# kalakris/stomp_motion_planner_icra2011

Measured on AMD Instinct MI355X. Metric: STOMP iterations/sec (7-DOF, 100 wp, K=512, 256³ SDF) at 1/2/4/8 GPUs, higher is better.
Workload: dtype f64; 1 GPU; cfg2: 7-DOF, 100 wp (N=99), K=512 (512/GPU), K_r=0, 256^3 SDF, S=49 spheres; global_rollouts=512, rollouts_per_gpu=512, parallelism=rollout shard x1

## Files before the change

stomp_motion_planner_icra2011_amd/csrc/device_fk.h:

```cpp
#pragma once

#include "kernels.h"
#include "stomp_math.h"

namespace stomp {

struct Frame {
    double R[9];
    double p[3];
};

__device__ __forceinline__ void rotmul(const double* A, const double* B, double* C)
{
#pragma unroll
    for (int i = 0; i < 3; ++i)
#pragma unroll
        for (int j = 0; j < 3; ++j)
            C[3 * i + j] = A[3 * i + 0] * B[0 + j] + A[3 * i + 1] * B[3 + j] + A[3 * i + 2] * B[6 + j];
}

__device__ __forceinline__ void pose_rotation(const DevSegment& sg, double st, double ct, double* R)
{
    const double* a = sg.axis;
    const double vt = 1.0 - ct;
    const double m_vt_0 = vt * a[0], m_vt_1 = vt * a[1], m_vt_2 = vt * a[2];
    const double m_st_0 = a[0] * st, m_st_1 = a[1] * st, m_st_2 = a[2] * st;
    const double m_vt_0_1 = m_vt_0 * a[1], m_vt_0_2 = m_vt_0 * a[2], m_vt_1_2 = m_vt_1 * a[2];
    double Rq[9];
    Rq[0] = ct + m_vt_0 * a[0];
    Rq[1] = -m_st_2 + m_vt_0_1;
    Rq[2] = m_st_1 + m_vt_0_2;
    Rq[3] = m_st_2 + m_vt_0_1;
    Rq[4] = ct + m_vt_1 * a[1];
    Rq[5] = -m_st_0 + m_vt_1_2;
    Rq[6] = -m_st_1 + m_vt_0_2;
    Rq[7] = m_st_0 + m_vt_1_2;
    Rq[8] = ct + m_vt_2 * a[2];
    if (sg.rot_identity) {
#pragma unroll
        for (int k = 0; k < 9; ++k) R[k] = Rq[k];
    } else {
#pragma unroll
        for (int i = 0; i < 3; ++i)
#pragma unroll
            for (int j = 0; j < 3; ++j)
                R[3 * i + j] = sg.rot[3 * i + 0] * Rq[0 + j] + sg.rot[3 * i + 1] * Rq[3 + j] + sg.rot[3 * i + 2] * Rq[6 + j];
    }
}

__device__ __forceinline__ void compose(const DevSegment& sg, const Frame* parent, double st, double ct, Frame& out)
{
    Frame pose;
    if (sg.q_index >= 0) {
        const double* a = sg.axis;
        const double vt = 1.0 - ct;
        const double m_vt_0 = vt * a[0], m_vt_1 = vt * a[1], m_vt_2 = vt * a[2];
        const double m_st_0 = a[0] * st, m_st_1 = a[1] * st, m_st_2 = a[2] * st;
        const double m_vt_0_1 = m_vt_0 * a[1], m_vt_0_2 = m_vt_0 * a[2], m_vt_1_2 = m_vt_1 * a[2];
        double Rq[9];
        Rq[0] = ct + m_vt_0 * a[0];
        Rq[1] = -m_st_2 + m_vt_0_1;
        Rq[2] = m_st_1 + m_vt_0_2;
        Rq[3] = m_st_2 + m_vt_0_1;
        Rq[4] = ct + m_vt_1 * a[1];
        Rq[5] = -m_st_0 + m_vt_1_2;
        Rq[6] = -m_st_1 + m_vt_0_2;
        Rq[7] = m_st_0 + m_vt_1_2;
        Rq[8] = ct + m_vt_2 * a[2];
        if (sg.rot_identity) {
#pragma unroll
            for (int k = 0; k < 9; ++k) pose.R[k] = Rq[k];
        } else {
            rotmul(sg.rot, Rq, pose.R);
        }
    } else {
#pragma unroll
        for (int k = 0; k < 9; ++k) pose.R[k] = sg.rot[k];
    }
#pragma unroll
    for (int k = 0; k < 3; ++k) pose.p[k] = sg.trans[k];
    if (!parent) {
        out = pose;
        return;
    }
    if (sg.q_index < 0 && sg.rot_identity) {
#pragma unroll
        for (int k = 0; k < 9; ++k) out.R[k] = parent->R[k];
    } else {
        rotmul(parent->R, pose.R, out.R);
    }
#pragma unroll
    for (int i = 0; i < 3; ++i)
        out.p[i] = parent->R[3 * i + 0] * pose.p[0] + parent->R[3 * i + 1] * pose.p[1] +
                   parent->R[3 * i + 2] * pose.p[2] + parent->p[i];
}

__device__ __forceinline__ void apply(const double* R, const double* P, const double* v, double* o)
{
#pragma unroll
    for (int i = 0; i < 3; ++i) o[i] = R[3 * i + 0] * v[0] + R[3 * i + 1] * v[1] + R[3 * i + 2] * v[2] + P[i];
}

__device__ __forceinline__ void fk_op(const DevSegment& sg, int base, int save, double st, double ct, Frame& C,
                                      Frame& S0, Frame& S1)
{
    Frame nf;
    if (base == kBaseChain) {
        compose(sg, &C, st, ct, nf);
    } else if (base == kBaseRoot) {
        compose(sg, nullptr, st, ct, nf);
    } else {
        Frame P;
#pragma unroll
        for (int k = 0; k < 9; ++k) P.R[k] = base == 0 ? S0.R[k] : S1.R[k];
#pragma unroll
        for (int k = 0; k < 3; ++k) P.p[k] = base == 0 ? S0.p[k] : S1.p[k];
        compose(sg, &P, st, ct, nf);
    }
    C = nf;
    if (save >= 0) {
#pragma unroll
        for (int k = 0; k < 9; ++k) {
            S0.R[k] = save == 0 ? C.R[k] : S0.R[k];
            S1.R[k] = save == 1 ? C.R[k] : S1.R[k];
        }
#pragma unroll
        for (int k = 0; k < 3; ++k) {
            S0.p[k] = save == 0 ? C.p[k] : S0.p[k];
            S1.p[k] = save == 1 ? C.p[k] : S1.p[k];
        }
    }
}

// ... 50 lines not shown
```

stomp_motion_planner_icra2011_amd/csrc/engine_create.cpp:

```cpp
#include "engine_internal.h"

#include <algorithm>
#include <cstdlib>

using namespace stomp;

namespace {

bool sphere_thresholds(double radius, double clearance, double res, int* zero_lim, int* col_lim)
{
    if (!(radius >= 0.0 && clearance > 0.0 && std::isfinite(radius) && std::isfinite(clearance))) return false;
    int zl = 65536, cl = 65536;
    bool zseen = false, cseen = false;
    for (int d2 = 0; d2 <= 65535; ++d2) {
        const double dist = std::sqrt((double)d2) * res;
        const double dd = dist - radius;
        const bool zero = dd >= clearance;
        const bool col = dist <= radius;
        if (zero && !zseen) { zl = d2; zseen = true; }
        if (!zero && zseen) return false;
        if (!col && !cseen) { cl = d2; cseen = true; }
        if (col && cseen) return false;
    }
    *zero_lim = zl;
    *col_lim = cl;
    return true;
}

int plan_fk(stomp_engine* e, const stomp_engine_desc* d, std::vector<FkOp>& ops)
{
    const int ns = d->num_segments;
    std::vector<char> needed(ns, 0);
    int prev = -1;
    for (int j = 0; j < d->num_spheres; ++j) {
        int s = d->spheres[j].segment;
        if (s < prev)
            return fail(e, STOMP_E_UNSUPPORTED,
                        "sphere list must be ordered by segment (sphere %d on segment %d after segment %d)", j, s, prev);
        prev = s;
        for (int a = s; a >= 0 && !needed[a]; a = d->segments[a].parent) needed[a] = 1;
    }
    std::vector<int> remaining(ns, 0), slot_of(ns, -1);
    for (int s = 0; s < ns; ++s)
        if (needed[s] && d->segments[s].parent >= 0) remaining[d->segments[s].parent]++;
    bool used[kSaves] = {false, false};
    const int runmax = run_max(d->num_time_steps);
    int sph = 0, cur = -1;
    for (int s = 0; s < ns; ++s) {
        if (!needed[s]) continue;
        const int p = d->segments[s].parent;
        int base;
        if (p < 0) base = kBaseRoot;
        else if (p == cur) base = kBaseChain;
        else if (slot_of[p] >= 0) base = slot_of[p];
        else return fail(e, STOMP_E_UNSUPPORTED, "FK planner: parent frame of segment %d not available", s);
        if (p >= 0 && --remaining[p] == 0 && slot_of[p] >= 0) {
            used[slot_of[p]] = false;
            slot_of[p] = -1;
        }
        int save = -1;
        if (remaining[s] >= 2) {
            for (int k = 0; k < kSaves; ++k)
                if (!used[k]) { used[k] = true; save = k; break; }
            if (save < 0) return fail(e, STOMP_E_UNSUPPORTED, "kinematic tree needs more than %d saved frames", kSaves);
            slot_of[s] = save;
        }
        cur = s;
        int b = sph;
        while (sph < d->num_spheres && d->spheres[sph].segment == s) ++sph;
        const int slot = sph > b ? e->nslots++ : -1;
        for (int j = b; j < sph; ++j) e->sphere_slot[j] = slot;
        bool first = true;
        for (int a = b; a < sph || first; a += runmax) {
            FkOp o;
            o.seg = first ? s : -1;
            o.base = first ? base : kBaseChain;
            o.save = first ? save : -1;
            o.slot = first ? slot : -1;
            o.sph_begin = std::min(a, sph);
            o.sph_end = std::min(a + runmax, sph);
            ops.push_back(o);
            first = false;
        }
    }
    return 0;
}

const char* torque_chain(const stomp_engine_desc* d, std::vector<int>& path)
{
    path.clear();
    if (!d->inertias) return "torque term needs segment inertias";
    if (d->torque_root < 0 || d->torque_root >= d->num_segments || d->torque_tip < 0 ||
        d->torque_tip >= d->num_segments)
        return "torque chain root/tip out of range";
    for (int sgi = d->torque_tip; sgi != d->torque_root; sgi = d->segments[sgi].parent) {
        if (sgi < 0 || (int)path.size() == kMaxChain) return "torque tip is not below the torque root (or chain too long)";
        path.push_back(sgi);
    }
    std::reverse(path.begin(), path.end());
    int nj = 0;
    for (int sgi : path)
        if (d->segments[sgi].q_index >= 0 && d->segments[sgi].q_index != nj++) return "torque chain joints must be the group joints in order";
    if (nj != d->num_joints) return "torque chain joints must be the group joints in order";
    return nullptr;
}

void oc_nominal_inverse(const double* q, double* O)
{
    double x = q[0], y = q[1], z = q[2], w = q[3];
    const double l2 = x * x + y * y + z * z + w * w;
    if (std::fabs(l2 - 1.0) > 0.1f) {
        const double inv = 1.0 / std::sqrt(l2);
        x *= inv; y *= inv; z *= inv; w *= inv;
    }
    const double d = x * x + y * y + z * z + w * w;
    const double s = 2.0 / d;
    const double xs = x * s, ys = y * s, zs = z * s;
    const double wx = w * xs, wy = w * ys, wz = w * zs;
    const double xx = x * xs, xy = x * ys, xz = x * zs;
    const double yy = y * ys, yz = y * zs, zz = z * zs;
    const double M[9] = {1.0 - (yy + zz), xy - wz, xz + wy, xy + wz, 1.0 - (xx + zz), yz - wx,
                         xz - wy, yz + wx, 1.0 - (xx + yy)};
    auto cof = [&](int r1, int c1, int r2, int c2) { return M[3 * r1 + c1] * M[3 * r2 + c2] - M[3 * r1 + c2] * M[3 * r2 + c1]; };
    const double co0 = cof(1, 1, 2, 2), co1 = cof(1, 2, 2, 0), co2 = cof(1, 0, 2, 1);
    const double det = M[0] * co0 + M[1] * co1 + M[2] * co2;
    const double sc = 1.0 / det;
    O[0] = co0 * sc; O[1] = cof(0, 2, 2, 1) * sc; O[2] = cof(0, 1, 1, 2) * sc;
    O[3] = co1 * sc; O[4] = cof(0, 0, 2, 2) * sc; O[5] = cof(0, 2, 1, 0) * sc;
    O[6] = co2 * sc; O[7] = cof(0, 1, 2, 0) * sc; O[8] = cof(0, 0, 1, 1) * sc;
}

struct HostTables {
    std::vector<double> LT, MT, QT;
    std::vector<DevSegment> segs;
    std::vector<DevSphere> sph;
    std::vector<int> slot_sph, has_lim;
    std::vector<double> jmin, jmax;
};

struct AbandonEngine {
    void operator()(stomp_engine* e) const
    {
        g_last_error = e->err;
        release(e);
        delete e;
    }
};

int world_of(const stomp_engine_desc* d) { return d->world_size > 0 ? d->world_size : 1; }

int validate_desc(const stomp_engine_desc* d)
{
    if (d->abi_version != STOMP_ENGINE_ABI_VERSION)
        return fail(nullptr, STOMP_E_INVALID, "abi_version %d != %d", d->abi_version, STOMP_ENGINE_ABI_VERSION);
    if (d->num_joints <= 0 || d->num_joints > kMaxJoints)
        return fail(nullptr, STOMP_E_INVALID, "num_joints must be in [1, %d]", kMaxJoints);
    if (d->num_time_steps <= 0 || d->num_time_steps > 256)
        return fail(nullptr, STOMP_E_INVALID, "num_time_steps must be in [1, 256]");
    if (d->num_rollouts <= 0) return fail(nullptr, STOMP_E_INVALID, "num_rollouts must be positive");
    if (d->num_reused_rollouts < 0 || d->num_reused_rollouts >= d->num_rollouts)
        return fail(nullptr, STOMP_E_INVALID, "Number of reused rollouts must be strictly less than number of rollouts.");
    if (d->num_orientation_constraints < 0 || (d->num_orientation_constraints > 0 && !d->orientation_constraints))
        return fail(nullptr, STOMP_E_INVALID, "invalid orientation constraints");
    for (int c = 0; c < d->num_orientation_constraints; ++c)
        if (d->orientation_constraints[c].segment < 0 || d->orientation_constraints[c].segment >= d->num_segments)
            return fail(nullptr, STOMP_E_INVALID, "orientation constraint %d: bad segment", c);
    if (d->num_segments <= 0 || !d->segments || (d->num_spheres > 0 && !d->spheres) || !d->joints || !d->noise_stddev ||
        !d->noise_decay || !d->start || !d->goal || !d->grid.data)
// ... 10 lines not shown
            return fail(nullptr, STOMP_E_INVALID, "sphere %d: bad segment", j);
        int zl, cl;
        if (!sphere_thresholds(d->spheres[j].radius, d->spheres[j].clearance, d->grid.resolution, &zl, &cl))
            return fail(nullptr, STOMP_E_INVALID, "sphere %d: radius / clearance not finite and positive", j);
    }
    if (d->torque_cost_weight > 1e-9) {
        std::vector<int> path;
        if (const char* why = torque_chain(d, path)) return fail(nullptr, STOMP_E_UNSUPPORTED, "%s", why);
    }
    const int world = world_of(d);
    if (world > 1) {
        if (!d->comm_id) return fail(nullptr, STOMP_E_INVALID, "world_size > 1 needs a comm_id");
        if (d->rank < 0 || d->rank >= world)
            return fail(nullptr, STOMP_E_INVALID, "rank %d outside [0, world_size %d)", d->rank, world);
        if (d->num_rollouts % (world * kSumBlock) != 0)
            return fail(nullptr, STOMP_E_INVALID, "num_rollouts must be a multiple of 64 * world_size");
        if (!kWithRccl && !is_local_comm_id(d->comm_id))
            return fail(nullptr, STOMP_E_UNSUPPORTED, "built without RCCL (use stomp_comm_local_id)");
    }
    return 0;
}

int open_engine(stomp_engine* e, const stomp_engine_desc* d)
{
    e->device = d->device;
    if (hipSetDevice(d->device) != hipSuccess) return fail(e, STOMP_E_DEVICE, "hipSetDevice(%d) failed", d->device);
    if (d->stream) {
        e->stream = (hipStream_t)d->stream;
    } else {
        hipStreamCreateWithFlags(&e->stream, hipStreamNonBlocking);
        e->own_stream = true;
    }
    const int world = world_of(d);
    e->J = d->num_joints; e->N = d->num_time_steps; e->Nall = e->N + 2 * kPad;
    e->K = d->num_rollouts; e->Kr = d->num_reused_rollouts;
    e->world = world; e->rank = world > 1 ? d->rank : 0;
    e->K_loc = e->K / world; e->first = e->rank * e->K_loc;
    e->S = d->num_spheres; e->nseg = d->num_segments; e->seed = d->seed;
    e->disc = d->discretization; e->w_smooth = d->smoothness_cost_weight; e->w_obs = d->obstacle_cost_weight;
    e->w_con = d->constraint_cost_weight; e->w_tq = d->torque_cost_weight;
    for (int r = 0; r < 3; ++r) e->smooth[r] = d->smoothness_costs[r];
    e->use_cum = d->use_cumulative_costs; e->max_it = d->max_iterations;
    e->max_it_cf = d->max_iterations_after_collision_free;
    e->sig_std.assign(d->noise_stddev, d->noise_stddev + e->J);
    e->sig_dec.assign(d->noise_decay, d->noise_decay + e->J);
    e->start.assign(d->start, d->start + e->J);
    e->goal.assign(d->goal, d->goal + e->J);
    return 0;
}

int choose_decomposition(stomp_engine* e, const stomp_engine_desc* d, bool local_id)
{
    const int world = e->world;
    if (e->K_loc > kSumBlock * 64) return fail(e, STOMP_E_INVALID, "at most %d rollouts per device", kSumBlock * 64);
    e->pre_on = (e->Kr == 0 || world == 1) && e->J <= 16;
    const bool can = e->pre_on && e->Kr == 0 && e->K <= kSumBlock * 64;
    const char* sm = std::getenv("STOMP_SHARD_MODE");
    if (world > 1 && sm && std::strcmp(sm, "gather") == 0 && !can)
        return fail(e, STOMP_E_UNSUPPORTED, "STOMP_SHARD_MODE=gather needs the pregen rows in the rollout launch "
                                            "and no reused rollouts (K_r = %d, J = %d)", e->Kr, e->J);
    const char* sim = std::getenv("STOMP_DEBUG_GATHER_RANKS");
    const int W = (world == 1 && sim) ? std::atoi(sim) : 0;
    if (W > 1 && can && e->K % (W * kSumBlock) == 0) {
        e->gather = true;
        e->K_loc = e->K / W;
    } else if (world > 1 && can) {
        e->gather = sm ? std::strcmp(sm, "gather") == 0 : (size_t)e->K * e->N * sizeof(double) <= (1u << 20);
    }
    const char* cl = std::getenv("STOMP_DEBUG_CALIBRATE_LOCAL");
    e->calibrate = world > 1 && can && !sm && (!local_id || (cl && cl[0] == '1'));
    if (e->calibrate) e->gather = true;
    e->rows = e->gather ? e->K : e->K_loc;
    e->row0 = (e->gather && world > 1) ? e->first : 0;
    const char* dbg = std::getenv("STOMP_DEBUG_SHARDED_MODES");
    e->split_modes = (world > 1 && !e->gather) ||
                     (world == 1 && !e->gather && dbg && dbg[0] == '1' && d->num_rollouts % kSumBlock == 0 &&
                      d->num_reused_rollouts == 0);
    return 0;
}

int setup_tables(stomp_engine* e, const stomp_engine_desc* d, HostTables& t)
{
    e->sphere_slot.assign(std::max(e->S, 1), 0);
    if (int rc = plan_fk(e, d, e->ops)) return rc;
    SetupInput si;
    si.J = e->J; si.N = e->N; si.discretization = e->disc;
    for (int r = 0; r < 3; ++r) si.smoothness_costs[r] = e->smooth[r];
    si.ridge_factor = d->ridge_factor;
    for (int j = 0; j < e->J; ++j) si.joint_cost.push_back(d->joints[j].joint_cost);
    si.start = e->start; si.goal = e->goal;
    std::string msg = compute_setup(si, e->su);
    if (!msg.empty()) return fail(e, STOMP_E_INVALID, "%s", msg.c_str());

    const int J = e->J, N = e->N;
    t.LT.assign((size_t)(N + kMatPadRows) * N, 0.0);
    t.MT.assign((size_t)(N + kMatPadRows) * N, 0.0);
    t.QT.resize((size_t)J * N * N);
    for (int i = 0; i < N; ++i)
        for (int k = 0; k < N; ++k) {
            t.LT[(size_t)k * N + i] = e->su.L[(size_t)i * N + k];
            t.MT[(size_t)k * N + i] = e->su.M[(size_t)i * N + k];
        }
    for (int j = 0; j < J; ++j)
        for (int i = 0; i < N; ++i)
            for (int k = 0; k < N; ++k)
                t.QT[((size_t)j * N + k) * N + i] = e->su.Qinv[((size_t)j * N + i) * N + k];
    t.segs.resize(e->nseg);
    for (int s = 0; s < e->nseg; ++s) {
        const stomp_segment& g = d->segments[s];
        DevSegment& o = t.segs[s];
        o.parent = g.parent; o.q_index = g.q_index;
        std::memcpy(o.rot, g.rot, sizeof g.rot);
        o.rot_identity = g.rot[0] == 1.0 && g.rot[1] == 0.0 && g.rot[2] == 0.0 && g.rot[3] == 0.0 &&
                         g.rot[4] == 1.0 && g.rot[5] == 0.0 && g.rot[6] == 0.0 && g.rot[7] == 0.0 &&
                         g.rot[8] == 1.0;
        o.pad_ = 0;
        std::memcpy(o.trans, g.trans, sizeof g.trans);
        std::memcpy(o.axis, g.axis, sizeof g.axis);
    }
    t.sph.resize(std::max(e->S, 1));
    for (int j = 0; j < e->S; ++j) {
        const stomp_sphere& g = d->spheres[j];
        DevSphere& o = t.sph[j];
        o.slot = e->sphere_slot[j];
        o.radius = g.radius; o.clearance = g.clearance;
        o.inv_clearance = 1.0 / g.clearance;
        std::memcpy(o.pos, g.pos, sizeof g.pos);
        sphere_thresholds(g.radius, g.clearance, d->grid.resolution, &o.zero_lim, &o.col_lim);
        o.pad_ = 0;
    }
    t.has_lim.resize(J);
    t.jmin.resize(J);
    t.jmax.resize(J);
    for (int j = 0; j < J; ++j) {
        t.has_lim[j] = d->joints[j].has_limits;
        t.jmin[j] = d->joints[j].min;
        t.jmax[j] = d->joints[j].max;
    }
    t.slot_sph.assign(e->nslots + 1, e->S);
    for (int j = e->S - 1; j >= 0; --j) t.slot_sph[e->sphere_slot[j]] = j;
    return 0;
}

int alloc_reuse_buffers(stomp_engine* e)
{
    const int J = e->J, N = e->N;
    if (e->world == 1 && e->Kr > 0) {
        if (int rc = dev_alloc(e, &e->d_reuse_costs, (size_t)e->K + 1)) return rc;
        if (int rc = dev_alloc(e, &e->d_reuse_count, 1)) return rc;
        const char* no_spec = std::getenv("STOMP_DEBUG_NO_SPEC");
        if (!(no_spec && std::strcmp(no_spec, "1") == 0)) {
            const size_t n = ((size_t)e->K + 1) * J * N;
            if (int rc = dev_alloc(e, &e->d_spec_params, n)) return rc;
            if (int rc = dev_alloc(e, &e->d_spec_noise, n)) return rc;
            if (int rc = dev_alloc(e, &e->d_spec_ctl, n)) return rc;
            e->spec_on = true;
        }
        const char* no_fuse = std::getenv("STOMP_DEBUG_NO_PICK_FUSE");
        e->pick_fuse = !(no_fuse && std::strcmp(no_fuse, "1") == 0);
    }
    if (e->world > 1 && e->Kr > 0) {
        const size_t slot = (size_t)e->Kr * ((size_t)J * N + N);
        if (int rc = dev_alloc(e, &e->d_tot_loc, (size_t)e->K_loc)) return rc;
        if (int rc = dev_alloc(e, &e->d_tot_all, (size_t)e->K)) return rc;
        if (int rc = dev_alloc(e, &e->d_tot_x, 1)) return rc;
        if (int rc = dev_alloc(e, &e->d_sel, (size_t)e->Kr)) return rc;
        if (int rc = dev_alloc(e, &e->d_slot, slot)) return rc;
        if (int rc = dev_alloc(e, &e->d_slot_all, slot * e->world)) return rc;
    }
    return 0;
}

int alloc_buffers(stomp_engine* e, const stomp_engine_desc* d, const HostTables& tab)
{
    const int J = e->J, N = e->N;
    if (int rc = upload(e, &e->d_QT, tab.QT.data(), tab.QT.size())) return rc;
    if (int rc = upload(e, &e->d_LT, tab.LT.data(), tab.LT.size())) return rc;
    if (int rc = upload(e, &e->d_MT, tab.MT.data(), tab.MT.size())) return rc;
    if (int rc = upload(e, &e->d_theta, e->su.theta.data(), e->su.theta.size())) return rc;
    if (int rc = upload(e, &e->d_start, e->start.data(), e->start.size())) return rc;
    if (int rc = upload(e, &e->d_goal, e->goal.data(), e->goal.size())) return rc;
    const size_t ncell = (size_t)d->grid.nx * d->grid.ny * d->grid.nz;
    e->grid_n[0] = d->grid.nx; e->grid_n[1] = d->grid.ny; e->grid_n[2] = d->grid.nz;
    if (d->grid.data_on_device) {
        e->d_sdf = (uint16_t*)d->grid.data;
        e->d_sdf_caller = d->grid.data;
    } else {
        if (int rc = upload(e, &e->d_sdf, d->grid.data, ncell)) return rc;
    }
    const size_t KJN = (size_t)e->rows * J * N;
    if (int rc = dev_alloc(e, &e->d_params, KJN)) return rc;
    if (int rc = dev_alloc(e, &e->d_noise, KJN)) return rc;
    if (int rc = dev_alloc(e, &e->d_control, KJN)) return rc;
    if (int rc = dev_alloc(e, &e->d_prob, KJN)) return rc;
    if (int rc = dev_alloc(e, &e->d_state, (size_t)e->rows * N)) return rc;
    if (e->gather && hipMemsetAsync(e->d_state, 0, sizeof(double) * e->rows * N, e->stream) != hipSuccess)
        return fail(e, STOMP_E_DEVICE, "memset failed");
    if (e->Kr > 0) {
        if (int rc = dev_alloc(e, &e->d_params_b, KJN)) return rc;
        if (int rc = dev_alloc(e, &e->d_noise_b, KJN)) return rc;
        if (int rc = dev_alloc(e, &e->d_control_b, KJN)) return rc;
        if (int rc = dev_alloc(e, &e->d_state_b, (size_t)e->K_loc * N)) return rc;
// ... 65 lines not shown
    t.torque = d->torque_cost_weight > 1e-9 ? 1 : 0;
    t.nchain = (int)cs.size();
    t.chain = d_chain;
    for (int k = 0; k < 3; ++k) t.g[k] = d->gravity[k];
    if (t.torque) e->terms_on = true;
    e->torque_stats = true;
    return 0;
}

int build_constraints(stomp_engine* e, const stomp_engine_desc* d)
{
    if (d->num_orientation_constraints <= 0) return 0;
    std::vector<OcDev> oc(d->num_orientation_constraints);
    for (int c = 0; c < d->num_orientation_constraints; ++c) {
        const stomp_orientation_constraint& in = d->orientation_constraints[c];
        OcDev& o = oc[c];
        std::vector<int> path;
        for (int sgi = in.segment; sgi >= 0; sgi = d->segments[sgi].parent) path.push_back(sgi);
        if ((int)path.size() > kMaxChain)
            return fail(e, STOMP_E_UNSUPPORTED, "constraint segment deeper than %d", kMaxChain);
        std::reverse(path.begin(), path.end());
        o.seg = in.segment; o.body_fixed = in.body_fixed ? 1 : 0; o.path_len = (int)path.size();
        for (size_t k = 0; k < path.size(); ++k) o.path[k] = path[k];
        oc_nominal_inverse(in.orientation, o.ninv);
        o.tol[0] = in.absolute_roll_tolerance; o.tol[1] = in.absolute_pitch_tolerance;
        o.tol[2] = in.absolute_yaw_tolerance; o.weight = in.weight;
        o.rw = o.pw = o.yw = 1.0;
        if (o.tol[1] >= M_PI) o.pw = 0.0;
        if (o.tol[0] >= M_PI) o.rw = 0.0;
        if (o.tol[2] >= M_PI) o.yw = 0.0;
    }
    OcDev* d_oc;
    if (int rc = upload(e, &d_oc, oc.data(), oc.size())) return rc;
    e->terms.noc = (int)oc.size();
    e->terms.oc = d_oc;
    e->terms_on = true;
    return 0;
}

int build_terms(stomp_engine* e, const stomp_engine_desc* d, const HostTables& tab)
{
    const int J = e->J, N = e->N;
    if (int rc = build_torque_chain(e, d, tab)) return rc;
    if (int rc = build_constraints(e, d)) return rc;
    if (e->terms_on || e->torque_stats) {
        TermsModel& t = e->terms;
        t.J = J; t.N = N;
        const double invTime = 1.0 / e->disc, invTime2 = 1.0 / (e->disc * e->disc);
        for (int k = 0; k < 7; ++k) {
            t.cv[k] = invTime * kDiffRules[0][k];
            t.ca[k] = invTime2 * kDiffRules[1][k];
        }
        t.start = e->d_start; t.goal = e->d_goal;
        t.w_con = e->w_con; t.w_tq = e->w_tq;
        if (terms_lds_bytes(t) > 160 * 1024) {
            if (e->terms_on)
                return fail(e, STOMP_E_UNSUPPORTED, "state-terms kernel needs %zu B of LDS", terms_lds_bytes(t));
            e->torque_stats = false;
        }
        if (getenv("STOMP_DEBUG_LEAN_PRINT"))
            fprintf(stderr, "stomp: terms J %d N %d nchain %d noc %d torque %d stats %d, k_terms<%d>, LDS %zu B, "
                            "opt-in %d\n", J, N, t.nchain, t.noc, t.torque, e->torque_stats ? 1 : 0, N <= 128 ? 128 : 256,
                    terms_lds_bytes(t), terms_lds_bytes(t) > 64 * 1024 ? 1 : 0);
        if (e->terms_on)
            if (int rc = dev_alloc(e, &e->d_terms_traj, (size_t)e->K_loc * J * N)) return rc;
        if (e->torque_stats) {
            e->tq_model = t;
            e->tq_model.torque = 1;
            e->tq_model.noc = 0;
            if (int rc = dev_alloc(e, &e->d_tq, (size_t)N)) return rc;
            if (int rc = dev_alloc(e, &e->d_tq_state, (size_t)N)) return rc;
        }
    }
    if (int rc = dev_alloc(e, &e->d_delta, (size_t)J * N)) return rc;
    e->pi_weight = e->w_smooth;
    if (hipDeviceGetAttribute(&e->wall_khz, hipDeviceAttributeWallClockRate, d->device) != hipSuccess) e->wall_khz = 0;
    return 0;
}

int choose_layout(stomp_engine* e, const stomp_engine_desc* d, const HostTables& tab)
{
    const int J = e->J, N = e->N;
    DevModel& m = e->model;
    m.J = J; m.N = N; m.Nall = e->Nall; m.S = e->S; m.nops = (int)e->ops.size(); m.nseg = e->nseg;
    m.nslots = e->nslots;
    m.sph_chunk = 1;
    for (const FkOp& o : e->ops) m.sph_chunk = std::max(m.sph_chunk, o.sph_end - o.sph_begin);
    if (m.sph_chunk * N > 65535)
        return fail(e, STOMP_E_UNSUPPORTED, "%d spheres on one segment x %d waypoints exceed 16-bit pair ids",
                    m.sph_chunk, N);
    m.nsaves = 0;
    for (const FkOp& o : e->ops) m.nsaves = std::max(m.nsaves, o.save + 1);
    int last_joint = -1, first_save = (int)e->ops.size();
    for (int i = 0; i < (int)e->ops.size(); ++i) {
        const FkOp& o = e->ops[i];
        if (o.seg >= 0 && tab.segs[o.seg].q_index >= 0) last_joint = i;
        if (o.save >= 0 && first_save == (int)e->ops.size()) first_save = i;
    }
    m.sincos_pre = m.nsaves >= 1 && J <= 12 * m.nsaves && first_save > last_joint ? 1 : 0;
    const size_t stat = rollout_static_lds();
    const size_t with_pad = rollout_lds_bytes(m, 1) + stat, without = rollout_lds_bytes(m, 0) + stat;
    int cus = 0;
    if (hipDeviceGetAttribute(&cus, hipDeviceAttributeMultiprocessorCount, d->device) != hipSuccess || cus <= 0)
        cus = 256;
    m.cus = cus;
    const int blocks = e->K_loc + 1 + (e->pre_on ? e->rows : 0) + (e->Kr > 0 && e->world == 1 ? e->K : 0);
    const int need = (blocks + cus - 1) / cus;
    m.pad_lds = (with_pad <= kRolloutLdsMax &&
                 rollout_blocks_per_cu(with_pad) >= std::min(need, rollout_blocks_per_cu(without))) ? 1 : 0;
    const size_t lds = rollout_lds_bytes(m, m.pad_lds) + stat;
    m.phased_lds = (int)rollout_phased_lds_bytes(m);
    if (getenv("STOMP_DEBUG_PHASED")) fprintf(stderr, "stomp: phased rollout LDS %d B\n", m.phased_lds);
    if (lds > kRolloutLdsMax)
        return fail(e, STOMP_E_UNSUPPORTED, "rollout kernel needs %zu B of LDS (J=%d, N=%d, S=%d, %d spheres "
                                            "on one segment), more than %zu", lds, J, N, e->S, m.sph_chunk,
                    kRolloutLdsMax);
    m.lean = 0;
    const int per_cu_full = rollout_blocks_per_cu(lds);
    int per_cu[3] = {per_cu_full, 0, 0};
    for (int lv = 1; lv <= 2; ++lv)
        if (rollout_lean_allowed(m, lv)) per_cu[lv] = rollout_blocks_per_cu(rollout_lds_bytes(m, 0, lv) + stat, lv);
    if (need > per_cu_full) {
        int best = per_cu_full;
        for (int lv = 1; lv <= 2; ++lv)
            if (per_cu[lv] > best) {
                best = per_cu[lv];
                m.lean = lv;
            }
    }
    if (const char* v = getenv("STOMP_DEBUG_LEAN")) {
        const int lv = atoi(v);
        if (lv >= 0 && lv <= 2 && rollout_lean_allowed(m, lv)) m.lean = lv;
    }
    if (getenv("STOMP_DEBUG_LEAN_PRINT"))
        fprintf(stderr, "stomp: rollout LDS full %zu / lean1 %zu / lean2 %zu B, workgroups per CU %d / %d / %d, "
                        "needed %d, layout lean %d\n", lds, rollout_lds_bytes(m, 0, 1) + stat,
                rollout_lds_bytes(m, 0, 2) + stat, per_cu[0], per_cu[1], per_cu[2], need, m.lean);
    if (!cost_supported(m)) return fail(e, STOMP_E_UNSUPPORTED, "FK program too large (%d ops, %d segments)",
                                        m.nops, m.nseg);
    return 0;
}

int upload_lds_image(stomp_engine* e, const HostTables& tab)
{
    const int J = e->J, N = e->N;
    DevModel& m = e->model;
    const RolloutLds L = rollout_lds(J, N, e->S, m.sph_chunk, m.nsaves, m.nseg, m.nops, m.nslots, 1);
    std::vector<unsigned char> img(L.total - L.sph, 0);
    auto put = [&](size_t off, const void* src, size_t bytes) {
        if (bytes) std::memcpy(img.data() + (off - L.sph), src, bytes);
    };
    std::vector<double> jlim(2 * (size_t)J);
    for (int j = 0; j < J; ++j) { jlim[2 * j] = tab.jmin[j]; jlim[2 * j + 1] = tab.jmax[j]; }
    put(L.sph, tab.sph.data(), sizeof(DevSphere) * e->S);
    put(L.seg, tab.segs.data(), sizeof(DevSegment) * tab.segs.size());
    put(L.ops, e->ops.data(), sizeof(FkOp) * e->ops.size());
    put(L.slot, tab.slot_sph.data(), sizeof(int) * tab.slot_sph.size());
    put(L.hl, tab.has_lim.data(), sizeof(int) * J);
    put(L.jlim, jlim.data(), sizeof(double) * jlim.size());
    unsigned long long* d_img;
    if (int rc = upload(e, &d_img, (const unsigned long long*)img.data(), img.size() / 8)) return rc;
    if (hipStreamSynchronize(e->stream) != hipSuccess)
        return fail(e, STOMP_E_DEVICE, "table upload failed");
    const unsigned char* base = (const unsigned char*)d_img;
    m.img = d_img;
    m.img_words = (int)(((m.pad_lds ? L.total : L.pad) - L.sph) / 8);
    m.sph = (const DevSphere*)(base + (L.sph - L.sph));
    m.segs = (const DevSegment*)(base + (L.seg - L.sph));
    m.ops = (const FkOp*)(base + (L.ops - L.sph));
    m.slot_sph = (const int*)(base + (L.slot - L.sph));
    e->d_pad_pos = (double*)(base + (L.pad - L.sph));
    m.pad_pos = e->d_pad_pos; m.sdf = e->d_sdf;
    return 0;
}

int place_field(stomp_engine* e, const stomp_engine_desc* d)
{
    DevModel& m = e->model;
    const size_t ncell = (size_t)d->grid.nx * d->grid.ny * d->grid.nz;
    const char* lay = std::getenv("STOMP_SDF_LAYOUT");
    const bool brick = lay ? std::strcmp(lay, "brick") == 0 : ncell * sizeof(uint16_t) > ((size_t)64 << 20);
    m.brick = 0;
    m.nby = (d->grid.ny + 3) / 4;
    m.nbz = (d->grid.nz + 3) / 4;
    if (!brick) return 0;
    uint16_t* bricks = nullptr;
    if (int rc = dev_alloc(e, &bricks, sdf_brick_cells(d->grid.nx, d->grid.ny, d->grid.nz))) return rc;
    launch_sdf_bricks(e->d_sdf, bricks, d->grid.nx, d->grid.ny, d->grid.nz, e->stream);
    if (hipStreamSynchronize(e->stream) != hipSuccess)
        return fail(e, STOMP_E_DEVICE, "distance-field brick layout failed");
    if (!d->grid.data_on_device) {
        auto it = std::find(e->allocs.begin(), e->allocs.end(), (void*)e->d_sdf);
        if (it != e->allocs.end()) {
            hipFree(*it);
            e->allocs.erase(it);
        }
    }
    e->d_sdf = bricks;
    m.sdf = bricks;
    m.brick = 1;
    return 0;
}

int finish_model(stomp_engine* e, const stomp_engine_desc* d)
{
    const int J = e->J, N = e->N;
    DevModel& m = e->model;
    e->terms.segs = m.segs;
    e->tq_model.segs = m.segs;
    m.nx = d->grid.nx; m.ny = d->grid.ny; m.nz = d->grid.nz;
    m.ny_d = (double)m.ny; m.nz_d = (double)m.nz;
    m.hi_x = m.nx - 1.5; m.hi_y = m.ny - 1.5; m.hi_z = m.nz - 1.5;
    m.ox = d->grid.origin[0]; m.oy = d->grid.origin[1]; m.oz = d->grid.origin[2]; m.res = d->grid.resolution;
    m.inv_res = 1.0 / d->grid.resolution;
    m.start = e->d_start; m.goal = e->d_goal;
    const double invTime = 1.0 / e->disc;
    for (int k = 0; k < 7; ++k) {
        m.vel_coef[k] = invTime * kDiffRules[0][k];
        if ((k < kVelTap0 || k > kVelTap1) && kDiffRules[0][k] != 0.0)
            return fail(e, STOMP_E_UNSUPPORTED, "velocity rule tap %d outside the kernel's stencil", k);
    }
    m.w_obs = e->w_obs; m.w_con = e->w_con; m.w_tq = e->w_tq;
    m.QT = e->d_QT;
    m.split_cap = std::max(e->K_loc + 2, m.cus / 2 + 1);
    if (int rc = dev_alloc(e, &m.split_cnt, (size_t)m.split_cap)) return rc;
    if (m.lean && m.nsaves > 0) {
        m.sv_rows = e->K_loc + 1;
        if (int rc = dev_alloc(e, &m.sv_glob, (size_t)m.sv_rows * m.nsaves * 12 * N)) return rc;
    }
    {
        const char* env = std::getenv("STOMP_DEBUG_SPLIT_MAX");
        m.split_max = env ? std::atoi(env) : 0;
        const char* xi = std::getenv("STOMP_DEBUG_XCTL_INLINE");
        m.x_ctl_inline = xi && std::strcmp(xi, "1") == 0 ? 1 : 0;
    }
    if (getenv("STOMP_DEBUG_LEAN_PRINT")) {
        const int nro = e->K_loc + 1, extra = e->pre_on ? e->rows : 0;
        const int P = rollout_split_pieces(m, nro, extra, false);
        const char* body = P ? "split" : nro <= m.cus ? (m.phased_lds > 0 ? "phased" : "wide")
                                                      : (m.lean ? "lean slot loop" : "slot loop");
        fprintf(stderr, "stomp: model J %d N %d S %d nseg %d nops %d nsaves %d sincos_pre %d sph_chunk %d lean %d "
                        "pregen %d fused_noise %d brick %d, launch of %d rollouts: %s, %d pieces, weights %s\n",
                J, N, e->S, m.nseg, m.nops, m.nsaves, m.sincos_pre, m.sph_chunk, m.lean, e->pre_on ? 1 : 0,
                J <= 16 ? 1 : 0, m.brick, nro, body, P, weights_kernel_name(e->K_loc, !e->split_modes, false));
    }
    return 0;
}

int pad_fk(stomp_engine* e)
{
    const int J = e->J, N = e->N;
    DevModel& m = e->model;
    m.pad_collision = 0;
    launch_pad_fk(m, e->d_start, e->d_goal, e->d_pad_pos, e->d_pad_cf, e->stream);
    int pad_cf = 0;
    if (hipMemcpyAsync(&pad_cf, e->d_pad_cf, sizeof(int), hipMemcpyDeviceToHost, e->stream) != hipSuccess ||
        hipStreamSynchronize(e->stream) != hipSuccess)
        return fail(e, STOMP_E_DEVICE, "padding FK failed: %s", hipGetErrorString(hipGetLastError()));
    m.pad_collision = pad_cf;
    e->pad_collision = pad_cf;
    if (hipMemcpyAsync(e->d_last_traj, e->d_theta, sizeof(double) * J * N, hipMemcpyDeviceToDevice, e->stream) !=
            hipSuccess ||
        hipMemcpyAsync(e->d_best_traj, e->d_theta, sizeof(double) * J * N, hipMemcpyDeviceToDevice, e->stream) !=
            hipSuccess)
        return fail(e, STOMP_E_DEVICE, "trajectory copies failed");
    return 0;
}

int settle_and_calibrate(stomp_engine* e)
{
    if (hipStreamSynchronize(e->stream) != hipSuccess) return fail(e, STOMP_E_DEVICE, "setup failed");
    return e->calibrate ? calibrate_shard_mode(e) : 0;
}

}

extern "C" int stomp_engine_create(const stomp_engine_desc* d, stomp_engine** out)
{
    if (!d || !out) return fail(nullptr, STOMP_E_INVALID, "null argument");
    *out = nullptr;
    if (int rc = validate_desc(d)) return rc;

    DeviceGuard dg(d->device);
    std::unique_ptr<stomp_engine, AbandonEngine> owner(new stomp_engine());
    stomp_engine* e = owner.get();
    const bool local_id = world_of(d) > 1 && is_local_comm_id(d->comm_id);
    HostTables tab;
    if (int rc = open_engine(e, d)) return rc;
    if (int rc = choose_decomposition(e, d, local_id)) return rc;
    if (int rc = setup_tables(e, d, tab)) return rc;
    if (int rc = alloc_buffers(e, d, tab)) return rc;
    if (int rc = build_terms(e, d, tab)) return rc;
    if (int rc = choose_layout(e, d, tab)) return rc;
    if (int rc = upload_lds_image(e, tab)) return rc;
    if (int rc = place_field(e, d)) return rc;
    if (int rc = finish_model(e, d)) return rc;
    if (int rc = pad_fk(e)) return rc;
    if (int rc = join_exchange(e, d->comm_id, local_id)) return rc;
    if (int rc = settle_and_calibrate(e)) return rc;
    *out = owner.release();
    return 0;
}
```

stomp_motion_planner_icra2011_amd/csrc/engine_internal.h:

```cpp
#pragma once

#include "stomp_engine.h"

#include <hip/hip_runtime.h>

#include <chrono>
#include <cmath>
#include <condition_variable>
#include <cstdarg>
#include <cstdio>
#include <cstring>
#include <memory>
#include <mutex>
#include <string>
#include <utility>
#include <vector>

#include "kernels.h"
#include "setup.h"

struct ncclComm;

namespace stomp {

enum TimerId { T_NOISE = 0, T_COST, T_WEIGHTS, T_UPDATE, T_NOISELESS, T_REUSE, T_TERMS, T_PREGEN, T_COUNT };
inline constexpr const char* kTimerNames[T_COUNT] = {"noise", "rollout_cost", "weights", "update", "noiseless", "reuse",
                                                     "state_terms", "pregen"};

struct LocalGroup {
    int world = 0;
    std::mutex mu;
    std::condition_variable cv;
    struct Slot {
        const void* src = nullptr;
        hipEvent_t ready = nullptr, done = nullptr;
        int device = 0;
    };
    std::vector<Slot> slot;
    std::vector<char> joined;
    long long phase = 0;
    int arrived = 0;
    bool has_sig = false;
    long long sig[6] = {0, 0, 0, 0, 0, 0};
    bool broken = false;
    bool barrier(std::unique_lock<std::mutex>& lk)
    {
        if (broken) return false;
        const long long my = phase;
        if (++arrived == world) {
            arrived = 0;
            ++phase;
            cv.notify_all();
            return true;
        }
        if (!cv.wait_for(lk, std::chrono::seconds(120), [&] { return phase != my || broken; }) || broken) {
            broken = true;
            cv.notify_all();
            return false;
        }
        return true;
    }
};

}

struct stomp_engine {
    std::string err;
    int device = 0;
    hipStream_t stream = nullptr;
    bool own_stream = false;
    int J = 0, N = 0, Nall = 0, K = 0, Kr = 0, K_loc = 0, first = 0, S = 0, nseg = 0;
    int world = 1, rank = 0;
    bool split_modes = false;
    bool gather = false;
    int rows = 0, row0 = 0;
    bool calibrate = false;
    double shard_info[6] = {0, 0, 0, 0, 0, 0};
    uint64_t seed = 0;
    double disc = 0.05, w_smooth = 0, w_obs = 0, w_con = 0, w_tq = 0;
    double smooth[3] = {0, 0, 0};
    int use_cum = 0, max_it = 0, max_it_cf = 0;
    std::vector<double> sig_std, sig_dec, start, goal;
    stomp::SetupOutput su;
    stomp::DevModel model{};
    stomp::TermsModel terms{};
    bool terms_on = false;
    double* d_terms_traj = nullptr;
    uint8_t* d_cs = nullptr;
    stomp::DevTrack* d_track = nullptr;
    const int* d_stop = nullptr;
    double* d_opt_costs = nullptr;
    stomp::DevTrack* h_track = nullptr;
    bool tracking = false;
    std::vector<stomp::FkOp> ops;
    std::vector<int> sphere_slot;
    int nslots = 0;
    std::vector<void*> allocs;
    double *d_theta = nullptr, *d_LT = nullptr, *d_MT = nullptr, *d_QT = nullptr;
    double *d_params = nullptr, *d_noise = nullptr, *d_control = nullptr, *d_prob = nullptr, *d_state = nullptr;
    double *d_params_b = nullptr, *d_noise_b = nullptr, *d_control_b = nullptr, *d_state_b = nullptr;
    int row_set = 0;
    double *d_cum = nullptr, *d_u = nullptr;
    double *d_x_params = nullptr, *d_x_noise = nullptr, *d_x_control = nullptr, *d_x_state = nullptr;
    double *d_last_traj = nullptr, *d_best_traj = nullptr, *d_total = nullptr;
    double *d_pad_pos = nullptr, *d_start = nullptr, *d_goal = nullptr;
    double *d_tot_loc = nullptr, *d_tot_all = nullptr, *d_tot_x = nullptr, *d_slot = nullptr, *d_slot_all = nullptr;
    double* d_reuse_costs = nullptr;
    int* d_reuse_count = nullptr;
    double *d_spec_params = nullptr, *d_spec_noise = nullptr, *d_spec_ctl = nullptr;
    bool spec_on = false;
    bool pick_fuse = true;
    int* d_sel = nullptr;
    uint8_t* d_cf = nullptr;
    uint16_t* d_sdf = nullptr;
    const uint16_t* d_sdf_caller = nullptr;
    int grid_n[3] = {0, 0, 0};
    int* d_pad_cf = nullptr;
    int pad_collision = 0;
    bool reused_next = false, extra_added = false;
    int pending_member = -1;
    double *d_mm = nullptr, *d_psum_part = nullptr, *d_psum_all = nullptr, *d_u_part = nullptr, *d_u_all = nullptr;
    int K_gen = 0;
    bool pre_on = false;
    int pre_it = -1;
    double *d_pre_eps[2] = {nullptr, nullptr}, *d_pre_meps[2] = {nullptr, nullptr};
    bool rows_in_pre = false;
    const double* rows_eps = nullptr;
    double* d_theta_gen = nullptr;
    double* h_total = nullptr;
    uint8_t* h_cf = nullptr;
    int eval_cap = 0;
    double *d_eval_params = nullptr, *d_eval_costs = nullptr, *d_eval_traj = nullptr;
    uint8_t* d_eval_cf = nullptr;
    uint8_t* d_eval_cs = nullptr;
    bool timing = false;
    struct Ev {
        int id;
        hipEvent_t a, b;
    };
    std::vector<Ev> evs;
    std::vector<hipEvent_t> pool;
    double tot_ms[stomp::T_COUNT] = {0};
    int launches[stomp::T_COUNT] = {0};
    ncclComm* comm = nullptr;
    const char* coll_name = "none";
    int coll_it = -1;
    long long coll_count = 0;
    int cur_it = -1;
    double comm_timeout_s = 300.0;
    bool comm_aborted = false;
    std::string comm_msg;
    long long stall_at = 0;
    unsigned* h_stall = nullptr;
    static constexpr int kCollRing = 32;
    struct CollRec {
        hipEvent_t ev = nullptr;
        const char* name = "";
        int it = -1;
        long long n = 0;
    } coll_ring[kCollRing];
    double pi_weight = 0.0;
    double* d_delta = nullptr;
    bool torque_stats = false;
    stomp::TermsModel tq_model{};
    double *d_tq = nullptr, *d_tq_state = nullptr;
    int wall_khz = 0;
    std::shared_ptr<stomp::LocalGroup> local;
    hipEvent_t ev_ready = nullptr, ev_done = nullptr;
    double* d_mm_all = nullptr;
};

namespace stomp {

extern thread_local std::string g_last_error;
int fail(stomp_engine* e, int code, const char* fmt, ...);
void release(stomp_engine* e);
void launch_noiseless(stomp_engine* e, int member);
int run_reuse(stomp_engine* e);

// ... 182 lines not shown
```

stomp_motion_planner_icra2011_amd/csrc/k_cost.hip:

```cpp
#include <algorithm>
#include <cassert>
#include <cstdlib>

#include "device_fk.h"
#include "limits_device.h"
#include "noise_device.h"
#include "stamps.h"

namespace stomp {

namespace {
constexpr int kMaxOps = 64;
constexpr int kMaxSeg = 64;
#ifndef ROLLOUT_BLOCK
#define ROLLOUT_BLOCK 256
#endif
constexpr int kBlock = ROLLOUT_BLOCK;
#ifndef ROLLOUT_MIN_WAVES
#define ROLLOUT_MIN_WAVES (ROLLOUT_BLOCK > 256 ? 4 : 3)
#endif
#ifndef ROLLOUT_WIDE_BLOCK
#define ROLLOUT_WIDE_BLOCK 512
#endif
constexpr int kWideBlock = ROLLOUT_WIDE_BLOCK;
#ifndef ROLLOUT_SPLIT_BLOCK
#define ROLLOUT_SPLIT_BLOCK 512
#endif
constexpr int kSplitBlock = ROLLOUT_SPLIT_BLOCK;
constexpr int kSplitMaxDefault = 6;
template <int BLOCK>
constexpr int rollout_min_waves()
{
    return BLOCK == kBlock ? ROLLOUT_MIN_WAVES : (BLOCK > 512 ? 4 : 2);
}
constexpr int kLaneSpheres = 8;
static_assert(kRunMaxSmall / 2 <= kLaneSpheres && kRunMaxLarge <= kLaneSpheres && kBlock >= 256,
              "a pair lane's spheres of one run must fit kLaneSpheres");
}

using CSegment = const __attribute__((address_space(4))) DevSegment;
using COp = const __attribute__((address_space(4))) FkOp;
using CSphere = const __attribute__((address_space(4))) DevSphere;
using CInt = const __attribute__((address_space(4))) int;
using CDouble = const __attribute__((address_space(4))) double;
__device__ __forceinline__ DevSegment load_seg(CSegment* p)
{
    DevSegment r;
    r.parent = p->parent;
    r.q_index = p->q_index;
    r.rot_identity = p->rot_identity;
    r.pad_ = 0;
#pragma unroll
    for (int k = 0; k < 9; ++k) r.rot[k] = p->rot[k];
#pragma unroll
    for (int k = 0; k < 3; ++k) {
        r.trans[k] = p->trans[k];
        r.axis[k] = p->axis[k];
    }
    return r;
}
__device__ __forceinline__ FkOp load_op(COp* p)
{
    FkOp r;
    r.seg = p->seg;
    r.base = p->base;
    r.save = p->save;
    r.sph_begin = p->sph_begin;
    r.sph_end = p->sph_end;
    r.slot = p->slot;
    return r;
}
__device__ __forceinline__ DevSphere load_sph(CSphere* p)
{
    DevSphere r;
    r.slot = p->slot;
    r.zero_lim = p->zero_lim;
    r.col_lim = p->col_lim;
    r.pad_ = 0;
    r.radius = p->radius;
    r.clearance = p->clearance;
    r.inv_clearance = p->inv_clearance;
#pragma unroll
    for (int k = 0; k < 3; ++k) r.pos[k] = p->pos[k];
    return r;
}
__device__ __forceinline__ double* global_ptr(double* p)
{
    return (double*)(__attribute__((address_space(1))) double*)p;
}

__device__ __forceinline__ void apply_lds(const double* fb, int N, int t, const double* pos, double* x)
{
#pragma unroll
    for (int i = 0; i < 3; ++i)
        x[i] = fb[(3 * i + 0) * N + t] * pos[0] + fb[(3 * i + 1) * N + t] * pos[1] +
               fb[(3 * i + 2) * N + t] * pos[2] + fb[(9 + i) * N + t];
// ... 1255 lines not shown
```

stomp_motion_planner_icra2011_amd/csrc/kernels.h:

```cpp
#pragma once

#include <hip/hip_runtime.h>
#include <stdint.h>

namespace stomp {

constexpr int kMaxJoints = 32;
constexpr int kRunMaxSmall = 16;
constexpr int kRunMaxLarge = 8;
constexpr int kSaves = 2;
constexpr int kSumBlock = 64;
constexpr int kBandBatch = 8;
constexpr int kMatPadRows = 16 * kBandBatch;
constexpr int kVelTap0 = 2;
constexpr int kVelTap1 = 5;
constexpr int kNoiseJT = 4;

inline int run_max(int N) { return N <= 128 ? kRunMaxSmall : kRunMaxLarge; }

constexpr int kBaseChain = -2;
constexpr int kBaseRoot = -1;

struct DevSegment {
    int parent, q_index;
    int rot_identity, pad_;
    double rot[9];
    double trans[3];
    double axis[3];
};

struct DevSphere {
    int slot;
    int zero_lim, col_lim, pad_;
    double radius, clearance, inv_clearance;
    double pos[3];
};

struct FkOp {
    int seg, base, save, sph_begin, sph_end;
    int slot;
};

struct DevModel {
    int J, N, Nall, S, nops, nseg, nslots, sph_chunk;
    int nsaves;
    int pad_lds;
    int sincos_pre;
    int cus;
    int phased_lds;
    const unsigned long long* img;
    int img_words;
    const DevSegment* segs;
    const DevSphere* sph;
    const FkOp* ops;
    const int* slot_sph;
    const double* pad_pos;
    const unsigned short* sdf;
    int nx, ny, nz;
    int brick;
    int nby, nbz;
    double ox, oy, oz, res, inv_res;
    double ny_d, nz_d;
    double hi_x, hi_y, hi_z;
    const double* start;
    const double* goal;
    double vel_coef[7];
    double w_obs, w_con, w_tq;
    int pad_collision;
    const double* QT;
    int* split_cnt;
    int split_cap;
    int split_max;
    int x_ctl_inline;
    int lean;
    double* sv_glob;
    int sv_rows;
};


struct RolloutLds {
    size_t traj, fb, sv, av, nzl, nzA, nzB, sph, seg, ops, slot, hl, jlim, pad, total;
};


__host__ __device__ inline size_t align16(size_t x) { return (x + 15) & ~(size_t)15; }

__host__ __device__ inline int noise_jp(int J) { return (J + kNoiseJT - 1) / kNoiseJT * kNoiseJT; }

__host__ __device__ inline RolloutLds rollout_lds(int J, int N, int S, int max_slot, int nsaves, int nseg, int nops,
                                                  int nslots, int pad_lds, bool phased = false, int lean = 0)
{
    RolloutLds l;
    if (phased) max_slot = S;
// ... 291 lines not shown
```

Measured before the change: 17310 iterations/s.

## Fold fixed root prefix into one synthetic segment and elide identity FK steps

The forward-kinematics planner now collapses the leading chain of fixed (non-joint) segments with no spheres into one precomposed synthetic root segment, computed on the host. It also drops chained fixed segments whose transform is exactly identity when nothing needs saving or sphere evaluation. The goal is to cut per-rollout, per-timestep frame compositions in the cost kernel. This adds a host-side compose path and an environment variable to disable folding, and it depends on the segment table layout accepting an extra appended segment.

```diff
diff --git a/stomp_motion_planner_icra2011_amd/csrc/device_fk.h b/stomp_motion_planner_icra2011_amd/csrc/device_fk.h
--- a/stomp_motion_planner_icra2011_amd/csrc/device_fk.h
+++ b/stomp_motion_planner_icra2011_amd/csrc/device_fk.h
@@ -10,7 +10,7 @@
     double p[3];
 };
 
-__device__ __forceinline__ void rotmul(const double* A, const double* B, double* C)
+__host__ __device__ __forceinline__ void rotmul(const double* A, const double* B, double* C)
 {
 #pragma unroll
     for (int i = 0; i < 3; ++i)
@@ -48,7 +48,7 @@
     }
 }
 
-__device__ __forceinline__ void compose(const DevSegment& sg, const Frame* parent, double st, double ct, Frame& out)
+__host__ __device__ __forceinline__ void compose(const DevSegment& sg, const Frame* parent, double st, double ct, Frame& out)
 {
     Frame pose;
     if (sg.q_index >= 0) {
diff --git a/stomp_motion_planner_icra2011_amd/csrc/engine_create.cpp b/stomp_motion_planner_icra2011_amd/csrc/engine_create.cpp
--- a/stomp_motion_planner_icra2011_amd/csrc/engine_create.cpp
+++ b/stomp_motion_planner_icra2011_amd/csrc/engine_create.cpp
@@ -1,4 +1,5 @@
 #include "engine_internal.h"
+#include "device_fk.h"
 
 #include <algorithm>
 #include <cstdlib>
@@ -27,9 +28,21 @@
     return true;
 }
 
-int plan_fk(stomp_engine* e, const stomp_engine_desc* d, std::vector<FkOp>& ops)
+int plan_fk(stomp_engine* e, const stomp_engine_desc* d, std::vector<FkOp>& ops, std::vector<int>& prefix)
 {
     const int ns = d->num_segments;
+    const char* nf = std::getenv("STOMP_DEBUG_NO_FK_FOLD");
+    const bool fold = !(nf && nf[0] == '1');
+    e->fk_steps_plain = e->fk_steps = 0;
+    prefix.clear();
+    bool in_prefix = fold && ns < kMaxSeg;
+    auto fixed_identity = [&](const stomp_segment& g) {
+        for (int k = 0; k < 9; ++k)
+            if (g.rot[k] != (k % 4 == 0 ? 1.0 : 0.0)) return false;
+        for (int k = 0; k < 3; ++k)
+            if (g.trans[k] != 0.0 || std::signbit(g.trans[k])) return false;
+        return g.q_index < 0;
+    };
     std::vector<char> needed(ns, 0);
     int prev = -1;
     for (int j = 0; j < d->num_spheres; ++j) {
@@ -46,9 +59,33 @@
     bool used[kSaves] = {false, false};
     const int runmax = run_max(d->num_time_steps);
     int sph = 0, cur = -1;
+    auto flush_prefix = [&]() {
+        in_prefix = false;
+        if (prefix.empty()) return;
+        FkOp o;
+        o.seg = prefix.size() >= 2 ? ns : prefix[0];
+        o.base = kBaseRoot;
+        o.save = o.slot = -1;
+        o.sph_begin = o.sph_end = sph;
+        ops.push_back(o);
+        ++e->fk_steps;
+        if (prefix.size() < 2) prefix.clear();
+    };
     for (int s = 0; s < ns; ++s) {
         if (!needed[s]) continue;
-        const int p = d->segments[s].parent;
+        ++e->fk_steps_plain;
+        const stomp_segment& g = d->segments[s];
+        const int p = g.parent;
+        if (in_prefix) {
+            const bool spheres = sph < d->num_spheres && d->spheres[sph].segment == s;
+            if (g.q_index < 0 && !spheres && remaining[s] == 1 && (prefix.empty() ? p < 0 : p == cur)) {
+                if (p >= 0) --remaining[p];
+                prefix.push_back(s);
+                cur = s;
+                continue;
+            }
+            flush_prefix();
+        }
         int base;
         if (p < 0) base = kBaseRoot;
         else if (p == cur) base = kBaseChain;
@@ -70,10 +107,13 @@
         while (sph < d->num_spheres && d->spheres[sph].segment == s) ++sph;
         const int slot = sph > b ? e->nslots++ : -1;
         for (int j = b; j < sph; ++j) e->sphere_slot[j] = slot;
+        const bool elide = fold && base == kBaseChain && save < 0 && fixed_identity(g);
+        if (elide && sph == b) continue;
+        if (!elide) ++e->fk_steps;
         bool first = true;
         for (int a = b; a < sph || first; a += runmax) {
             FkOp o;
-            o.seg = first ? s : -1;
+            o.seg = first && !elide ? s : -1;
             o.base = first ? base : kBaseChain;
             o.save = first ? save : -1;
             o.slot = first ? slot : -1;
@@ -83,7 +123,24 @@
             first = false;
         }
     }
-    return 0;
+    if (in_prefix) flush_prefix();
+    return 0;
+}
+
+DevSegment synthetic_root(const std::vector<DevSegment>& segs, const std::vector<int>& prefix)
+{
+    Frame C, nf;
+    compose(segs[prefix[0]], nullptr, 0.0, 1.0, C);
+    for (size_t i = 1; i < prefix.size(); ++i) {
+        compose(segs[prefix[i]], &C, 0.0, 1.0, nf);
+        C = nf;
+    }
+    DevSegment o;
+    o.parent = -1; o.q_index = -1; o.rot_identity = 0; o.pad_ = 0;
+    std::memcpy(o.rot, C.R, sizeof o.rot);
+    std::memcpy(o.trans, C.p, sizeof o.trans);
+    o.axis[0] = 0.0; o.axis[1] = 0.0; o.axis[2] = 1.0;
+    return o;
 }
 
 const char* torque_chain(const stomp_engine_desc* d, std::vector<int>& path)
@@ -260,7 +317,8 @@
 int setup_tables(stomp_engine* e, const stomp_engine_desc* d, HostTables& t)
 {
     e->sphere_slot.assign(std::max(e->S, 1), 0);
-    if (int rc = plan_fk(e, d, e->ops)) return rc;
+    std::vector<int> prefix;
+    if (int rc = plan_fk(e, d, e->ops, prefix)) return rc;
     SetupInput si;
     si.J = e->J; si.N = e->N; si.discretization = e->disc;
     for (int r = 0; r < 3; ++r) si.smoothness_costs[r] = e->smooth[r];
@@ -296,6 +354,7 @@
         std::memcpy(o.trans, g.trans, sizeof g.trans);
         std::memcpy(o.axis, g.axis, sizeof g.axis);
     }
+    if (prefix.size() >= 2) t.segs.push_back(synthetic_root(t.segs, prefix));
     t.sph.resize(std::max(e->S, 1));
     for (int j = 0; j < e->S; ++j) {
         const stomp_sphere& g = d->spheres[j];
@@ -527,7 +586,8 @@
 {
     const int J = e->J, N = e->N;
     DevModel& m = e->model;
-    m.J = J; m.N = N; m.Nall = e->Nall; m.S = e->S; m.nops = (int)e->ops.size(); m.nseg = e->nseg;
+    m.J = J; m.N = N; m.Nall = e->Nall; m.S = e->S; m.nops = (int)e->ops.size();
+    m.nseg = (int)tab.segs.size();
     m.nslots = e->nslots;
     m.sph_chunk = 1;
     for (const FkOp& o : e->ops) m.sph_chunk = std::max(m.sph_chunk, o.sph_end - o.sph_begin);
@@ -688,6 +748,7 @@
                         "pregen %d fused_noise %d brick %d, launch of %d rollouts: %s, %d pieces, weights %s\n",
                 J, N, e->S, m.nseg, m.nops, m.nsaves, m.sincos_pre, m.sph_chunk, m.lean, e->pre_on ? 1 : 0,
                 J <= 16 ? 1 : 0, m.brick, nro, body, P, weights_kernel_name(e->K_loc, !e->split_modes, false));
+        fprintf(stderr, "stomp: fk steps %d folded to %d\n", e->fk_steps_plain, e->fk_steps);
     }
     return 0;
 }
diff --git a/stomp_motion_planner_icra2011_amd/csrc/engine_internal.h b/stomp_motion_planner_icra2011_amd/csrc/engine_internal.h
--- a/stomp_motion_planner_icra2011_amd/csrc/engine_internal.h
+++ b/stomp_motion_planner_icra2011_amd/csrc/engine_internal.h
@@ -95,6 +95,7 @@
     std::vector<stomp::FkOp> ops;
     std::vector<int> sphere_slot;
     int nslots = 0;
+    int fk_steps_plain = 0, fk_steps = 0;
     std::vector<void*> allocs;
     double *d_theta = nullptr, *d_LT = nullptr, *d_MT = nullptr, *d_QT = nullptr;
     double *d_params = nullptr, *d_noise = nullptr, *d_control = nullptr, *d_prob = nullptr, *d_state = nullptr;
diff --git a/stomp_motion_planner_icra2011_amd/csrc/k_cost.hip b/stomp_motion_planner_icra2011_amd/csrc/k_cost.hip
--- a/stomp_motion_planner_icra2011_amd/csrc/k_cost.hip
+++ b/stomp_motion_planner_icra2011_amd/csrc/k_cost.hip
@@ -11,7 +11,6 @@
 
 namespace {
 constexpr int kMaxOps = 64;
-constexpr int kMaxSeg = 64;
 #ifndef ROLLOUT_BLOCK
 #define ROLLOUT_BLOCK 256
 #endif
diff --git a/stomp_motion_planner_icra2011_amd/csrc/kernels.h b/stomp_motion_planner_icra2011_amd/csrc/kernels.h
--- a/stomp_motion_planner_icra2011_amd/csrc/kernels.h
+++ b/stomp_motion_planner_icra2011_amd/csrc/kernels.h
@@ -9,6 +9,7 @@
 constexpr int kRunMaxSmall = 16;
 constexpr int kRunMaxLarge = 8;
 constexpr int kSaves = 2;
+constexpr int kMaxSeg = 64;
 constexpr int kSumBlock = 64;
 constexpr int kBandBatch = 8;
 constexpr int kMatPadRows = 16 * kBandBatch;
```

After: 17350 iterations/s, median of 6. About the same (+0.2%).
